# taohan10200/CRA5

Hardware: AMD Instinct MI355X
Metric: ERA5 frames/s (721x1440x268) encode+decode (higher is better)
Workload: dtype f32 (3xf16-split MFMA, fp32 accumulate)

## Files before the change

cra5_amd/csrc/attention_split_f16.hip:

```cpp
#include <hip/hip_runtime.h>
#include <math.h>
#include <stdlib.h>

#include "../../include/cra5_amd.h"
#include "split.h"

CRA5_RANGE_TU(attn)

typedef float f32x16 __attribute__((ext_vector_type(16)));
typedef _Float16 half8 __attribute__((ext_vector_type(8)));
typedef _Float16 half4 __attribute__((ext_vector_type(4)));
typedef __fp16 fp16x4 __attribute__((__vector_size__(4 * sizeof(__fp16))));
#if defined(__HIP_DEVICE_COMPILE__)
#define CRA5_TR_READ(P) \
  __builtin_bit_cast(half4, __builtin_amdgcn_ds_read_tr16_b64_v4f16((__attribute__((address_space(3))) fp16x4 *)(P)))
#else
#define CRA5_TR_READ(P) (*reinterpret_cast<const half4 *>(P))
#endif

namespace {

__device__ __forceinline__ int xcd_remap(int bid, int nb) {
  const int q = nb / 8, r = nb % 8;
  const int xcd = bid % 8, within = bid / 8;
  const int base = (xcd < r) ? xcd * (q + 1) : r * (q + 1) + (xcd - r) * q;
  return base + within;
}

struct WinGeom {
  int H, W, wh, ww, nwc;
};

__device__ __forceinline__ int token_of(const WinGeom &g, int wr, int wc, int t) {
  if (g.ww == g.W && g.wh == g.H) return t;
  const int r = t / g.ww, c = t - r * g.ww;
  const int gr = wr * g.wh + r, gc = wc * g.ww + c;
  return (gr < g.H && gc < g.W) ? gr * g.W + gc : -1;
}

#ifdef CRA5_ATTN_TRACE
__device__ unsigned long long g_attn_trace[6 * 8192];
#define CRA5_ATRACE(SLOT, VAL)                                                                          \
  if (threadIdx.x == 0 && atrace_idx < 8192) g_attn_trace[atrace_idx * 6 + (SLOT)] = (VAL);
#else
#define CRA5_ATRACE(SLOT, VAL)
#endif

constexpr int HD = 64;
constexpr int KS = 72;
constexpr int VS = 96;
constexpr int MAX_WIN_TOKENS = 1152;

struct BalArgs {
  int groups;
  int n_full;
  int n_wg_pass;
  int rem_tile0;
  int rem;
  int n_grp;
  int nkt;
  int maxp;
  float *ws;
};
__host__ __device__ __forceinline__ long bal_cut(long S, int G, int c) { return S * c / G; }
__host__ __device__ __forceinline__ int bal_piece_of(long S, int G, long s) {
  int c = (int)(s * G / S);
  if (c > G - 1) c = G - 1;
  while (c > 0 && bal_cut(S, G, c) > s) --c;
  while (c < G - 1 && bal_cut(S, G, c + 1) <= s) ++c;
  return c;
}
constexpr int WS_ROW = 68;

template <int NW, bool HI, bool GLOBAL, bool BAL = false, bool PLAIN = false>
__global__ __launch_bounds__(NW * 64, (NW >= 8 ? 1 : (NW == 4 ? 3 : 2))) void window_attention_split_kernel(
    const unsigned short *__restrict__ qkv, long ldq ,
    const unsigned short *__restrict__ pad_row, float *__restrict__ out, unsigned short *__restrict__ out_s,
    int Kp_out, int C, int heads, WinGeom g, int q_tiles , float scale, BalArgs bal) {
  static_assert(!BAL || GLOBAL, "the balanced schedule is for whole-grid launches");
  static_assert(!PLAIN || HI, "plain rows carry no lo plane");
  constexpr int NT = NW * 64;
  constexpr int PPR = PLAIN ? 8 : 16;
  constexpr int PIECES = 32 * PPR;
  constexpr int STG = (PIECES + NT - 1) / NT;

  constexpr int KPL = 32 * KS + 32;
  constexpr int VPL = 32 * VS;
  constexpr int KBUF = 2 * KPL, VBUF = 2 * VPL;
  __shared__ __attribute__((aligned(16))) unsigned short lds[2 * KBUF + 2 * VBUF];
  unsigned short *Ks = lds;
  unsigned short *Vt = lds + 2 * KBUF;
  constexpr int TAB = GLOBAL ? 1 : MAX_WIN_TOKENS;
  __shared__ long long tab[TAB];

  const int L = g.wh * g.ww;
  int head, win, n_seg = 1;
  int seg_tile0[2] = {0, 0}, seg_nact[2] = {NW, NW}, seg_j0[2] = {0, 0}, seg_j1[2] = {L / 32, L / 32}, seg_part[2] = {-1, -1};
  int seg_grp[2] = {0, 0};
  if (BAL) {
    const int pass = blockIdx.x / bal.n_wg_pass, w = blockIdx.x - pass * bal.n_wg_pass;
    int slot;
    if ((heads & 7) == 0 && (bal.n_wg_pass & 7) == 0) {
      const int xcd = w & 7, s_ = w >> 3;
      head = xcd * (heads >> 3) + s_ / bal.groups;
      slot = s_ % bal.groups;
    } else {
      head = w / bal.groups;
      slot = w % bal.groups;
    }
    win = 0;
    if (pass < bal.n_full) {
      seg_tile0[0] = (pass * bal.groups + slot) * NW;
    } else {
      const long S = (long)bal.n_grp * bal.nkt;
      const long s0 = bal_cut(S, bal.groups, slot), s1 = bal_cut(S, bal.groups, slot + 1);
      n_seg = 0;
      for (long s = s0; s < s1;) {
        const int gq = (int)(s / bal.nkt);
        const long e = min(s1, (long)(gq + 1) * bal.nkt);
        if (n_seg < 2) {
          seg_grp[n_seg] = gq;
          seg_tile0[n_seg] = bal.rem_tile0 + gq * NW;
          seg_nact[n_seg] = min(NW, bal.rem - gq * NW);
          seg_j0[n_seg] = (int)(s - (long)gq * bal.nkt);
          seg_j1[n_seg] = (int)(e - (long)gq * bal.nkt);
          seg_part[n_seg] = slot - bal_piece_of(S, bal.groups, (long)gq * bal.nkt);
          ++n_seg;
        }
        s = e;
      }
    }
  } else {
    const int pid = xcd_remap(blockIdx.x, gridDim.x);
    const int qt = pid % q_tiles;
    const int wh_id = pid / q_tiles;
    head = wh_id % heads;
    win = wh_id / heads;
    seg_tile0[0] = qt * NW;
  }
  const int wr = win / g.nwc, wc = win - wr * g.nwc;

  const int tid = threadIdx.x, lane = tid & 63, wave = tid >> 6;
  const int l31 = lane & 31, h = lane >> 5;
  const int hoff = head * HD;
  const long qoff = (PLAIN ? 1L : 2L) * hoff, koff = (PLAIN ? 1L : 2L) * (C + hoff), voff = (PLAIN ? 1L : 2L) * (2 * C + hoff);

  if (!GLOBAL) {
    const long long pad_delta = reinterpret_cast<const char *>(pad_row) - reinterpret_cast<const char *>(qkv);
    for (int t = tid; t < L; t += NT) {
      const int tok = token_of(g, wr, wc, t);
      tab[t] = (tok >= 0) ? (long long)tok * ldq * 2 : pad_delta;
    }
  }
  constexpr bool IDLE_SKIP = !GLOBAL || BAL;
  bool tab_ready = GLOBAL;
#pragma unroll 1
  for (int seg = 0; seg < n_seg; ++seg) {
  const int tile0 = seg_tile0[seg], n_active = seg_nact[seg], j0 = seg_j0[seg], j1 = seg_j1[seg];
#ifdef CRA5_ATTN_TRACE
  const int atrace_idx = GLOBAL ? 8192 : (int)blockIdx.x;
  const unsigned long long atrace_c0 = clock64();
#endif
  CRA5_ATRACE(0, wall_clock64());
  const int tq = (tile0 + wave) * 32 + l31;
  const int q_tok = (tq < L && wave < n_active) ? token_of(g, wr, wc, tq) : -1;
  const bool wave_active = __any(q_tok >= 0);
  if (!__syncthreads_or(wave_active ? 1 : 0)) continue;
  tab_ready = true;

  half8 qh[4], ql[4];
  {
    const unsigned short *qrow = ((q_tok >= 0) ? qkv + (size_t)q_tok * ldq : pad_row) + qoff;
#pragma unroll
    for (int s = 0; s < 4; ++s) {
      const int chunk = s >> 1, pp = 2 * (s & 1) + h;
      if (PLAIN) {
        qh[s] = *reinterpret_cast<const half8 *>(qrow + 16 * s + 8 * h);
        ql[s] = qh[s];
      } else {
        qh[s] = *reinterpret_cast<const half8 *>(qrow + chunk * 64 + pp * 8);
        ql[s] = *reinterpret_cast<const half8 *>(qrow + chunk * 64 + 32 + pp * 8);
      }
    }
  }
  const float cexp = scale * 1.44269504088896340736f;
  f32x16 negm;
#pragma unroll
  for (int r = 0; r < 16; ++r) negm[r] = 0.f;
  if (HI) {
#pragma unroll
    for (int s = 0; s < 4; ++s)
#pragma unroll
      for (int e = 0; e < 8; ++e) qh[s][e] = (_Float16)((float)qh[s][e] * cexp);
  }
  const float cmax = HI ? 1.0f : cexp;

  f32x16 o[2];
#pragma unroll
  for (int t = 0; t < 2; ++t)
#pragma unroll
    for (int r = 0; r < 16; ++r) o[t][r] = 0.f;
  float m_run = HI ? 0.f : -INFINITY, l_run = 0.f;

  const int n_tiles = j1 - j0;
  uint4 sk0 = make_uint4(0u, 0u, 0u, 0u), sk1 = sk0, sv0 = sk0, sv1 = sk0;
  static_assert(STG == 1 || STG == 2, "staging below is written out for one or two 16-byte pieces per thread");
  constexpr bool TWO = STG == 2;
  const int krow0 = min(tid / PPR, 31), krow1 = min((tid + NT) / PPR, 31);
  const long kcol = koff + (tid % PPR) * 8;
  const long vcol = voff + (tid % PPR) * 8;
  const unsigned short *kq0 = qkv + (size_t)(krow0 + 32 * j0) * ldq + kcol;
  const unsigned short *kq1 = qkv + (size_t)(krow1 + 32 * j0) * ldq + kcol;
  const unsigned short *vq0 = qkv + (size_t)(krow0 + 32 * j0) * ldq + vcol;
  const unsigned short *vq1 = qkv + (size_t)(krow1 + 32 * j0) * ldq + vcol;
  const long tile_step = 32 * ldq;
#define CRA5_ROW(JJ, ROW) \
  reinterpret_cast<const unsigned short *>(reinterpret_cast<const char *>(qkv) + tab[(JJ)*32 + (ROW)])
  const bool stage0 = (NT <= PIECES) || (tid < PIECES);
  const bool stage1 = TWO && (tid + NT < PIECES);
#define CRA5_K_LOAD(J)                                                                    \
  if (stage0) {                                                                           \
    if (GLOBAL) {                                                                         \
      sk0 = *reinterpret_cast<const uint4 *>(kq0);                                        \
      if (stage1) sk1 = *reinterpret_cast<const uint4 *>(kq1);                            \
      const long st_ = ((J) < n_tiles - 1) ? tile_step : 0;  \
      kq0 += st_;                                                                         \
      kq1 += st_;                                                                         \
    } else {                                                                              \
      const int jj_ = min((J), n_tiles - 1);                                              \
      sk0 = *reinterpret_cast<const uint4 *>(CRA5_ROW(jj_, krow0) + kcol);                \
      if (stage1) sk1 = *reinterpret_cast<const uint4 *>(CRA5_ROW(jj_, krow1) + kcol);    \
    }                                                                                     \
  }
#define CRA5_V_LOAD(J)                                                                    \
  if (stage0) {                                                                           \
    if (GLOBAL) {                                                                         \
      sv0 = *reinterpret_cast<const uint4 *>(vq0);                                        \
      if (stage1) sv1 = *reinterpret_cast<const uint4 *>(vq1);                            \
      const long st_ = ((J) < n_tiles - 1) ? tile_step : 0;                               \
      vq0 += st_;                                                                         \
      vq1 += st_;                                                                         \
    } else {                                                                              \
      const int jj_ = min((J), n_tiles - 1);                                              \
      sv0 = *reinterpret_cast<const uint4 *>(CRA5_ROW(jj_, krow0) + vcol);                \
      if (stage1) sv1 = *reinterpret_cast<const uint4 *>(CRA5_ROW(jj_, krow1) + vcol);    \
    }                                                                                     \
  }
#define CRA5_K_STORE1(P, BUF)                                                             \
  {                                                                                       \
    const int idx = tid + (P)*NT;                                                         \
    if (idx < PIECES) {                                                                   \
      const int row = idx / PPR, piece = idx % PPR;                                       \
      const int plane = PLAIN ? 0 : (piece >> 2) & 1, d0 = PLAIN ? 8 * piece : 32 * (piece >> 3) + 8 * (piece & 3); \
      *reinterpret_cast<uint4 *>(Ks + (BUF)*KBUF + plane * KPL + row * KS + d0) = sk##P;  \
    }                                                                                     \
  }
#define CRA5_K_STORE(BUF) { CRA5_K_STORE1(0, BUF) if (TWO) CRA5_K_STORE1(1, BUF) }
#define CRA5_V_STORE1(P, BUF)                                                             \
  {                                                                                       \
    const int idx = tid + (P)*NT;                                                         \
    if (idx < PIECES) {                                                                   \
      const int row = idx / PPR, piece = idx % PPR;                                       \
      const int plane = PLAIN ? 0 : (piece >> 2) & 1, d0 = PLAIN ? 8 * piece : 32 * (piece >> 3) + 8 * (piece & 3); \
      *reinterpret_cast<uint4 *>(Vt + (BUF)*VBUF + plane * VPL + row * VS + d0) = sv##P;  \
    }                                                                                     \
  }
#define CRA5_V_STORE(BUF) { CRA5_V_STORE1(0, BUF) if (TWO) CRA5_V_STORE1(1, BUF) }
#define CRA5_SCORES(DST, KB)                                                              \
  {                                                                                       \
    f32x16 acc_;                                                                          \
    _Pragma("unroll") for (int r = 0; r < 16; ++r) acc_[r] = 0.f;                         \
    _Pragma("unroll") for (int st = 0; st < 4; ++st) {                                    \
      const half8 kh = *reinterpret_cast<const half8 *>(k_base + (KB)*KBUF + 16 * st);     \
      const half8 kl = *reinterpret_cast<const half8 *>(k_base + (KB)*KBUF + KPL + 16 * st); \
      if (!HI) {                                                                          \
        acc_ = __builtin_amdgcn_mfma_f32_32x32x16_f16(kl, qh[st], acc_, 0, 0, 0);         \
        acc_ = __builtin_amdgcn_mfma_f32_32x32x16_f16(kh, ql[st], acc_, 0, 0, 0);         \
      }                                                                                   \
      if (HI && st == 0) {                                                                \
        CRA5_MFMA_FROM(acc_, kh, qh[0], negm);                                            \
      } else {                                                                            \
        acc_ = __builtin_amdgcn_mfma_f32_32x32x16_f16(kh, qh[st], acc_, 0, 0, 0);         \
      }                                                                                   \
    }                                                                                     \
    DST = acc_;                                                                           \
  }
#if defined(__HIP_DEVICE_COMPILE__)
#define CRA5_MFMA_FROM(D, A, B, C) \
  asm("s_nop 3\n\tv_mfma_f32_32x32x16_f16 %0, %1, %2, %3" : "=&v"(D) : "v"(A), "v"(B), "v"(C))
#else
#define CRA5_MFMA_FROM(D, A, B, C) (D) = (C)
#endif

  const unsigned short *k_base = Ks + l31 * KS + 8 * h;
  const unsigned short *v_base = Vt + (4 * h + ((lane & 15) >> 2)) * VS + 16 * ((lane >> 4) & 1) + 4 * (lane & 3);

#if defined(__HIP_DEVICE_COMPILE__)
#define CRA5_XHALF_MAX(X)                                                                 \
  ({                                                                                      \
    float a_ = (X), b_ = (X), r_;                                                         \
    asm("s_nop 1\n\tv_permlane32_swap_b32_e32 %0, %1\n\ts_nop 1\n\tv_max_f32_e32 %2, %0, %1" \
        : "+v"(a_), "+v"(b_), "=v"(r_));                                                  \
    r_;                                                                                   \
  })
#define CRA5_MAX2_VALU(A, B)                                                              \
  ({                                                                                      \
    float r_;                                                                             \
    asm("v_max_f32_e32 %0, %1, %2" : "=v"(r_) : "v"(A), "v"(B));                          \
    r_;                                                                                   \
  })
#else
#define CRA5_XHALF_MAX(X) (X)
#define CRA5_MAX2_VALU(A, B) fmaxf((A), (B))
#endif
#if !defined(__HIP_DEVICE_COMPILE__)
#define CRA5_TILE_MAX(S)                                                                  \
  ({                                                                                      \
    float m_ = fmaxf(fmaxf(fmaxf(S[0], S[1]), fmaxf(S[2], S[3])), fmaxf(fmaxf(S[4], S[5]), fmaxf(S[6], S[7]))); \
    float n_ = fmaxf(fmaxf(fmaxf(S[8], S[9]), fmaxf(S[10], S[11])), fmaxf(fmaxf(S[12], S[13]), fmaxf(S[14], S[15]))); \
    CRA5_XHALF_MAX(fmaxf(m_, n_)) * cmax;       \
  })
#else
#define CRA5_MAX3(A, B, C) fmaxf(fmaxf((A), (B)), (C))
#define CRA5_TILE_MAX(S)                                                                  \
  ({                                                                                      \
    const float a_ = CRA5_MAX3(S[0], S[1], S[2]), b_ = CRA5_MAX3(S[3], S[4], S[5]), c_ = CRA5_MAX3(S[6], S[7], S[8]); \
    const float d_ = CRA5_MAX3(S[9], S[10], S[11]), e_ = CRA5_MAX3(S[12], S[13], S[14]);     \
    const float f_ = CRA5_MAX3(a_, b_, c_), g_ = CRA5_MAX3(d_, e_, S[15]);                   \
    CRA5_XHALF_MAX(CRA5_MAX2_VALU(f_, g_)) * cmax;  \
  })
#endif

  f32x16 s_cur;
  CRA5_K_LOAD(0);
  CRA5_V_LOAD(0);
  CRA5_K_STORE(0);
  CRA5_V_STORE(0);
  CRA5_K_LOAD(1);
  CRA5_K_STORE(1);
  __syncthreads();
  CRA5_K_LOAD(2);
  CRA5_V_LOAD(1);
  CRA5_SCORES(s_cur, 0);
  float mloc = CRA5_TILE_MAX(s_cur);
  __syncthreads();

  auto key_tile = [&](const int j, f32x16 &s_cur, f32x16 &s_next) __attribute__((always_inline)) {
    const int kb = (j + 1) & 1, vb = j & 1;
    if (!IDLE_SKIP || wave_active) {
    constexpr float DEFER_LOG2 = 8.0f;
    auto shift = [&](float delta, const bool rescale, f32x16 *also) __attribute__((always_inline)) {
      delta = (float)(_Float16)fminf(fmaxf(delta, -60000.f), 60000.f);
      if (rescale) {
        const float alpha = __builtin_amdgcn_exp2f(-delta);
        l_run *= alpha;
#pragma unroll
        for (int t = 0; t < 2; ++t)
#pragma unroll
          for (int r = 0; r < 16; ++r) o[t][r] *= alpha;
      }
      m_run += delta;
      half8 e0, bd;
#pragma unroll
      for (int e = 0; e < 8; ++e) {
        e0[e] = (_Float16)0.0f;
        bd[e] = (_Float16)0.0f;
      }
      e0[0] = (_Float16)(h == 0 ? 1.0f : 0.0f);
      bd[0] = (_Float16)(h == 0 ? -delta : 0.0f);
      s_cur = __builtin_amdgcn_mfma_f32_32x32x16_f16(e0, bd, s_cur, 0, 0, 0);
      negm = __builtin_amdgcn_mfma_f32_32x32x16_f16(e0, bd, negm, 0, 0, 0);
      if (also) *also = __builtin_amdgcn_mfma_f32_32x32x16_f16(e0, bd, *also, 0, 0, 0);
#if defined(__HIP_DEVICE_COMPILE__)
      asm volatile("s_nop 15\n\ts_nop 3" ::: "memory");
#endif
    };
    if (HI) {
      if (j == 0) shift(mloc, false, nullptr);
    } else if (!__all(mloc - m_run <= DEFER_LOG2)) {
      const float m_new = fmaxf(m_run, mloc);
      const float alpha = __builtin_amdgcn_exp2f(m_run - m_new);
      l_run *= alpha;
#pragma unroll
      for (int t = 0; t < 2; ++t)
#pragma unroll
        for (int r = 0; r < 16; ++r) o[t][r] *= alpha;
      m_run = m_new;
    }
    const float m_new = m_run;
#if defined(__HIP_DEVICE_COMPILE__)
    if (!HI) {
#define CRA5_FENCE() __builtin_amdgcn_sched_barrier(0)
#define CRA5_STAGE(MFMA_STMT) \
  CRA5_FENCE();               \
  MFMA_STMT;                  \
  CRA5_FENCE();
#define CRA5_KFRAG(PLANE, ST) (*reinterpret_cast<const half8 *>(k_base + kb * KBUF + (PLANE)*KPL + 16 * (ST)))
#define CRA5_MM(A, B, C) __builtin_amdgcn_mfma_f32_32x32x16_f16((A), (B), (C), 0, 0, 0)
      typedef _Float16 half2v __attribute__((ext_vector_type(2)));
      typedef unsigned u32x4 __attribute__((ext_vector_type(4)));
      float p[16], psum = 0.f;
      u32x4 phw[2], plw[2];
      auto exp_half = [&](const int u) __attribute__((always_inline)) {
        p[2 * u] = __builtin_amdgcn_exp2f(fmaf(s_cur[2 * u], cexp, -m_new));
        p[2 * u + 1] = __builtin_amdgcn_exp2f(fmaf(s_cur[2 * u + 1], cexp, -m_new));
      };
      auto split_half = [&](const int u) __attribute__((always_inline)) {
        const int r = 2 * u;
        const half2v h2 = {(_Float16)p[r], (_Float16)p[r + 1]};
        const unsigned hh = __builtin_bit_cast(unsigned, h2);
        float d0, d1;
        asm("v_fma_mix_f32 %0, %2, -1.0, %3 op_sel_hi:[1,0,0]\n\t"
            "v_fma_mix_f32 %1, %2, -1.0, %4 op_sel:[1,0,0] op_sel_hi:[1,0,0]"
            : "=&v"(d0), "=&v"(d1) : "v"(hh), "v"(p[r]), "v"(p[r + 1]));
        psum += p[r];
        psum += p[r + 1];
        const half2v l2 = {(_Float16)d0, (_Float16)d1};
        unsigned ll = __builtin_bit_cast(unsigned, l2);
        asm("" : "+v"(ll));
        phw[u >> 2][u & 3] = hh;
        plw[u >> 2][u & 3] = ll;
      };
#define ph(T) __builtin_bit_cast(half8, phw[T])
#define pl(T) __builtin_bit_cast(half8, plw[T])
      half8 vh[2], vl[2];
      auto v_frag = [&](const int t, const int plane, const int dt) __attribute__((always_inline)) {
        const unsigned short *vp = v_base + vb * VBUF + plane * VPL + 16 * t * VS + 32 * dt;
        const half4 a0 = CRA5_TR_READ(vp);
        const half4 a1 = CRA5_TR_READ(vp + 8 * VS);
        return __builtin_shufflevector(a0, a1, 0, 1, 2, 3, 4, 5, 6, 7);
      };
      half8 kh0 = CRA5_KFRAG(0, 0), kl0 = CRA5_KFRAG(1, 0), kh1 = CRA5_KFRAG(0, 1), kl1 = CRA5_KFRAG(1, 1);
      f32x16 acc;
#pragma unroll
      for (int r = 0; r < 16; ++r) acc[r] = 0.f;
      CRA5_STAGE(acc = CRA5_MM(kl0, qh[0], acc))
      exp_half(0);
      CRA5_STAGE(acc = CRA5_MM(kh0, ql[0], acc))
      exp_half(1);
      CRA5_STAGE(acc = CRA5_MM(kh0, qh[0], acc))
      split_half(0);
      const half8 kh2 = CRA5_KFRAG(0, 2), kl2 = CRA5_KFRAG(1, 2);
      CRA5_STAGE(acc = CRA5_MM(kl1, qh[1], acc))
      exp_half(2);
      CRA5_STAGE(acc = CRA5_MM(kh1, ql[1], acc))
      split_half(1);
      CRA5_STAGE(acc = CRA5_MM(kh1, qh[1], acc))
      exp_half(3);
      const half8 kh3 = CRA5_KFRAG(0, 3), kl3 = CRA5_KFRAG(1, 3);
      CRA5_STAGE(acc = CRA5_MM(kl2, qh[2], acc))
      split_half(2);
      CRA5_STAGE(acc = CRA5_MM(kh2, ql[2], acc))
      exp_half(4);
      CRA5_STAGE(acc = CRA5_MM(kh2, qh[2], acc))
      split_half(3);
      CRA5_STAGE(acc = CRA5_MM(kl3, qh[3], acc))
      exp_half(5);
      vl[0] = v_frag(0, 1, 0);
      vl[1] = v_frag(0, 1, 1);
      CRA5_STAGE(acc = CRA5_MM(kh3, ql[3], acc))
      split_half(4);
      CRA5_STAGE(acc = CRA5_MM(kh3, qh[3], acc))
      split_half(5);
      vh[0] = v_frag(0, 0, 0);
      vh[1] = v_frag(0, 0, 1);
      s_next = acc;
      CRA5_STAGE(o[0] = CRA5_MM(vl[0], ph(0), o[0]))
      exp_half(6);
      CRA5_STAGE(o[1] = CRA5_MM(vl[1], ph(0), o[1]))
      exp_half(7);
      CRA5_STAGE(o[0] = CRA5_MM(vh[0], pl(0), o[0]))
      split_half(6);
      CRA5_STAGE(o[1] = CRA5_MM(vh[1], pl(0), o[1]))
      split_half(7);
      vl[0] = v_frag(1, 1, 0);
      vl[1] = v_frag(1, 1, 1);
      CRA5_STAGE(o[0] = CRA5_MM(vh[0], ph(0), o[0]))
      l_run += psum;
      CRA5_STAGE(o[1] = CRA5_MM(vh[1], ph(0), o[1]))
      vh[0] = v_frag(1, 0, 0);
      vh[1] = v_frag(1, 0, 1);
      CRA5_STAGE(o[0] = CRA5_MM(vl[0], ph(1), o[0]))
      const float ma = CRA5_MAX3(s_next[0], s_next[1], s_next[2]), mb = CRA5_MAX3(s_next[3], s_next[4], s_next[5]);
      const float mc = CRA5_MAX3(s_next[6], s_next[7], s_next[8]), md = CRA5_MAX3(s_next[9], s_next[10], s_next[11]);
      const float me = CRA5_MAX3(s_next[12], s_next[13], s_next[14]);
      CRA5_STAGE(o[1] = CRA5_MM(vl[1], ph(1), o[1]))
      const float mf = CRA5_MAX3(ma, mb, mc), mg = CRA5_MAX3(md, me, s_next[15]);
      const float mfg = CRA5_MAX2_VALU(mf, mg);
      CRA5_STAGE(o[0] = CRA5_MM(vh[0], pl(1), o[0]))
      const float mx = CRA5_XHALF_MAX(mfg);
      CRA5_STAGE(o[1] = CRA5_MM(vh[1], pl(1), o[1]))
      mloc = mx * cmax;
      CRA5_STAGE(o[0] = CRA5_MM(vh[0], ph(1), o[0]))
      CRA5_STAGE(o[1] = CRA5_MM(vh[1], ph(1), o[1]))
#undef ph
#undef pl
#undef CRA5_MM
#undef CRA5_KFRAG
#undef CRA5_STAGE
#undef CRA5_FENCE
    } else
#endif
    {
    CRA5_SCORES(s_next, kb);
    float psum = 0.f;
    half8 ph[2], pl[2];
#if defined(__HIP_DEVICE_COMPILE__)
    if (HI) {
      typedef _Float16 half2v __attribute__((ext_vector_type(2)));
      typedef _Float16 half8v __attribute__((ext_vector_type(8)));
      const half2v ones = {(_Float16)1.0f, (_Float16)1.0f};
      auto exps = [&]() __attribute__((always_inline)) {
        psum = 0.f;
#pragma unroll
        for (int t = 0; t < 2; ++t) {
          half2v hp[4];
#pragma unroll
          for (int i = 0; i < 4; ++i) {
            hp[i] = half2v{(_Float16)__builtin_amdgcn_exp2f(s_cur[8 * t + 2 * i]), (_Float16)__builtin_amdgcn_exp2f(s_cur[8 * t + 2 * i + 1])};
            psum = __builtin_amdgcn_fdot2(hp[i], ones, psum, false);
          }
          ph[t] = half8v{hp[0][0], hp[0][1], hp[1][0], hp[1][1], hp[2][0], hp[2][1], hp[3][0], hp[3][1]};
        }
      };
      exps();
      constexpr float P_SAFE = 8192.0f;
      if (!__all(psum <= P_SAFE)) {
        const float mrel = CRA5_TILE_MAX(s_cur);
        shift(fmaxf(mrel, 0.f), true, &s_next);
        exps();
      }
#pragma unroll
      for (int t = 0; t < 2; ++t)
#pragma unroll
        for (int e = 0; e < 8; ++e) pl[t][e] = (_Float16)0.0f;
    }
#else
#pragma unroll
    for (int r = 0; r < 16; ++r) {
      const float p = HI ? (float)(_Float16)__builtin_amdgcn_exp2f(s_cur[r]) : __builtin_amdgcn_exp2f(fmaf(s_cur[r], cexp, -m_new));
      psum += p;
      const _Float16 hi = (_Float16)p;
      const _Float16 lo = (_Float16)(p - (float)hi);
      ph[r >> 3][r & 7] = hi;
      pl[r >> 3][r & 7] = lo;
    }
#endif
    l_run += psum;
#pragma unroll
    for (int t = 0; t < 2; ++t) {
      half8 vh[2], vl[2];
#pragma unroll
      for (int dt = 0; dt < 2; ++dt) {
        const unsigned short *vp = v_base + vb * VBUF + 16 * t * VS + 32 * dt;
        const unsigned short *vq = vp + VPL;
        const half4 a0 = CRA5_TR_READ(vp);
        const half4 a1 = CRA5_TR_READ(vp + 8 * VS);
        const half4 b0 = CRA5_TR_READ(vq);
        const half4 b1 = CRA5_TR_READ(vq + 8 * VS);
        vh[dt] = __builtin_shufflevector(a0, a1, 0, 1, 2, 3, 4, 5, 6, 7);
        vl[dt] = __builtin_shufflevector(b0, b1, 0, 1, 2, 3, 4, 5, 6, 7);
      }
      if (!HI) {
        o[0] = __builtin_amdgcn_mfma_f32_32x32x16_f16(vl[0], ph[t], o[0], 0, 0, 0);
        o[1] = __builtin_amdgcn_mfma_f32_32x32x16_f16(vl[1], ph[t], o[1], 0, 0, 0);
        o[0] = __builtin_amdgcn_mfma_f32_32x32x16_f16(vh[0], pl[t], o[0], 0, 0, 0);
        o[1] = __builtin_amdgcn_mfma_f32_32x32x16_f16(vh[1], pl[t], o[1], 0, 0, 0);
      }
      o[0] = __builtin_amdgcn_mfma_f32_32x32x16_f16(vh[0], ph[t], o[0], 0, 0, 0);
      o[1] = __builtin_amdgcn_mfma_f32_32x32x16_f16(vh[1], ph[t], o[1], 0, 0, 0);
    }
    if (!HI) mloc = CRA5_TILE_MAX(s_next);
    }
    }
    CRA5_K_STORE(j & 1);
    CRA5_V_STORE((j + 1) & 1);
    CRA5_K_LOAD(j + 3);
    CRA5_V_LOAD(j + 2);
    __syncthreads();
  };
  CRA5_ATRACE(1, wall_clock64());
  f32x16 s_alt;
  const int n_loop = n_tiles;
  int jt = 0;
  for (; jt + 1 < n_loop; jt += 2) {
    key_tile(jt, s_cur, s_alt);
    key_tile(jt + 1, s_alt, s_cur);
  }
  if (jt < n_loop) key_tile(jt, s_cur, s_alt);
  CRA5_ATRACE(2, wall_clock64());
  CRA5_ATRACE(4, (unsigned long long)n_tiles);

  const float l_tot = l_run + __shfl_xor(l_run, 32, 64);
  if (BAL && seg_part[seg] >= 0) {
    if (q_tok >= 0) {
      float *wrow = bal.ws + (((((size_t)head * bal.n_grp + seg_grp[seg]) * bal.maxp + seg_part[seg]) * NW + wave) * 32 + l31) * WS_ROW;
#pragma unroll
      for (int t = 0; t < 2; ++t)
#pragma unroll
        for (int gq = 0; gq < 4; ++gq) {
          const int d = 32 * t + 8 * gq + 4 * h;
          *reinterpret_cast<float4 *>(wrow + d) = make_float4(o[t][4 * gq + 0], o[t][4 * gq + 1], o[t][4 * gq + 2], o[t][4 * gq + 3]);
        }
      if (h == 0) {
        wrow[64] = m_run;
        wrow[65] = l_tot;
      }
    }
    continue;
  }
  {
    const bool live = q_tok >= 0;
    const float inv = live ? 1.0f / l_tot : 0.0f;
    float *orow = (out && live) ? out + (size_t)q_tok * C + hoff : nullptr;
    unsigned short *srow = (out_s && live) ? out_s + (size_t)q_tok * 2 * Kp_out : nullptr;
#pragma unroll
    for (int t = 0; t < 2; ++t)
#pragma unroll
      for (int pr = 0; pr < 2; ++pr) {
        float va[4], vb[4];
#pragma unroll
        for (int k = 0; k < 4; ++k) {
          va[k] = o[t][4 * (2 * pr) + k] * inv;
          vb[k] = o[t][4 * (2 * pr + 1) + k] * inv;
        }
        if (orow) {
          *reinterpret_cast<float4 *>(orow + 32 * t + 16 * pr + 4 * h) = make_float4(va[0], va[1], va[2], va[3]);
          *reinterpret_cast<float4 *>(orow + 32 * t + 16 * pr + 8 + 4 * h) = make_float4(vb[0], vb[1], vb[2], vb[3]);
        }
        if (out_s) {
          unsigned ha0, la0, ha1, la1, hb0, lb0, hb1, lb1;
          cra5_split_pair(va[0], va[1], ha0, la0);
          cra5_split_pair(va[2], va[3], ha1, la1);
          cra5_split_pair(vb[0], vb[1], hb0, lb0);
          cra5_split_pair(vb[2], vb[3], hb1, lb1);
#if defined(__HIP_DEVICE_COMPILE__)
#define CRA5_SWAP32(A, B)                                                  \
  {                                                                        \
    const auto r_ = __builtin_amdgcn_permlane32_swap((A), (B), false, false); \
    (A) = r_[0];                                                           \
    (B) = r_[1];                                                           \
  }
          CRA5_SWAP32(ha0, hb0);
          CRA5_SWAP32(ha1, hb1);
          CRA5_SWAP32(la0, lb0);
          CRA5_SWAP32(la1, lb1);
#undef CRA5_SWAP32
#endif
          if (srow) {
            const int c0 = hoff + 32 * t + 16 * pr + 8 * h;
            unsigned short *sp = srow + (PLAIN ? c0 : (c0 >> 5) * 64 + (c0 & 31));
            *reinterpret_cast<uint4 *>(sp) = make_uint4(ha0, ha1, hb0, hb1);
            if (!HI) *reinterpret_cast<uint4 *>(sp + 32) = make_uint4(la0, la1, lb0, lb1);
          }
        }
      }
  }
  CRA5_ATRACE(3, wall_clock64());
  CRA5_ATRACE(5, clock64() - atrace_c0);
  }
  (void)tab_ready;
}

__global__ __launch_bounds__(256) void attention_merge_kernel(const float *__restrict__ ws, float *__restrict__ out,
                                                              unsigned short *__restrict__ out_s, int Kp_out, int C,
                                                              BalArgs bal, int nw, int plain) {
  const int t = blockIdx.x % nw, hg = blockIdx.x / nw;
  const int grp = hg % bal.n_grp, head = hg / bal.n_grp;
  if (grp * nw + t >= bal.rem) return;
  const long S = (long)bal.n_grp * bal.nkt;
  const int c0 = bal_piece_of(S, bal.groups, (long)grp * bal.nkt);
  const int c1 = bal_piece_of(S, bal.groups, (long)(grp + 1) * bal.nkt - 1);
  const int np = c1 - c0 + 1;
  const int q = threadIdx.x >> 3, d0 = (threadIdx.x & 7) * 8;
  const size_t pstride = (size_t)nw * 32 * WS_ROW;
  const float *base = ws + ((((size_t)head * bal.n_grp + grp) * bal.maxp) * nw + t) * 32 * WS_ROW + (size_t)q * WS_ROW;
  float M = -INFINITY;
  for (int c = 0; c < np; ++c) M = fmaxf(M, base[c * pstride + 64]);
  float acc[8] = {0.f, 0.f, 0.f, 0.f, 0.f, 0.f, 0.f, 0.f}, lsum = 0.f;
  for (int c = 0; c < np; ++c) {
    const float *r = base + c * pstride;
    const float a = __builtin_amdgcn_exp2f(r[64] - M);
    lsum = fmaf(r[65], a, lsum);
    const float4 v0 = *reinterpret_cast<const float4 *>(r + d0), v1 = *reinterpret_cast<const float4 *>(r + d0 + 4);
    acc[0] = fmaf(v0.x, a, acc[0]);
    acc[1] = fmaf(v0.y, a, acc[1]);
    acc[2] = fmaf(v0.z, a, acc[2]);
    acc[3] = fmaf(v0.w, a, acc[3]);
    acc[4] = fmaf(v1.x, a, acc[4]);
    acc[5] = fmaf(v1.y, a, acc[5]);
    acc[6] = fmaf(v1.z, a, acc[6]);
    acc[7] = fmaf(v1.w, a, acc[7]);
  }
  const float inv = 1.0f / lsum;
  const int tok = (bal.rem_tile0 + grp * nw + t) * 32 + q, col = head * HD + d0;
#pragma unroll
  for (int k = 0; k < 8; ++k) acc[k] *= inv;
  if (out) {
    *reinterpret_cast<float4 *>(out + (size_t)tok * C + col) = make_float4(acc[0], acc[1], acc[2], acc[3]);
    *reinterpret_cast<float4 *>(out + (size_t)tok * C + col + 4) = make_float4(acc[4], acc[5], acc[6], acc[7]);
  }
  if (out_s) {
    unsigned short *srow = out_s + (size_t)tok * 2 * Kp_out;
    if (plain) {
      cra5_store_plain4(srow, col, acc[0], acc[1], acc[2], acc[3]);
      cra5_store_plain4(srow, col + 4, acc[4], acc[5], acc[6], acc[7]);
    } else {
      cra5_store_split4(srow, col, acc[0], acc[1], acc[2], acc[3]);
      cra5_store_split4(srow, col + 4, acc[4], acc[5], acc[6], acc[7]);
    }
  }
}

int cu_count() {
  static const int n = [] {
    int dev = 0, v = 0;
    if (hipGetDevice(&dev) != hipSuccess) return 256;
    if (hipDeviceGetAttribute(&v, hipDeviceAttributeMultiprocessorCount, dev) != hipSuccess || v <= 0) return 256;
    return v;
  }();
  return n;
}

constexpr int NW_GLOBAL = 12;

bool balanced_plan(int L, int heads, BalArgs &b) {
  const int P = cu_count(), T = L / 32;
  if (P % heads) return false;
  b.groups = P / heads;
  b.n_full = T / (b.groups * NW_GLOBAL);
  b.rem_tile0 = b.n_full * b.groups * NW_GLOBAL;
  b.rem = T - b.rem_tile0;
  b.n_grp = (b.rem + NW_GLOBAL - 1) / NW_GLOBAL;
  b.nkt = T;
  b.n_wg_pass = heads * b.groups;
  b.ws = nullptr;
  b.maxp = 0;
  const long S = (long)b.n_grp * b.nkt;
  for (int g = 0; g < b.n_grp; ++g) {
    const int np = bal_piece_of(S, b.groups, (long)(g + 1) * b.nkt - 1) - bal_piece_of(S, b.groups, (long)g * b.nkt) + 1;
    if (np > b.maxp) b.maxp = np;
  }
  if (!(b.n_full >= 1 && (b.rem == 0 || (b.n_grp <= b.groups && S >= b.groups)))) return false;
  for (int c = 0; b.rem && c < b.groups; ++c) {
    const long s0 = bal_cut(S, b.groups, c), s1 = bal_cut(S, b.groups, c + 1);
    if (s1 > s0 && (s1 - 1) / b.nkt - s0 / b.nkt + 1 > 2) return false;
  }
  return true;
}

size_t balanced_ws_bytes(const BalArgs &b, int heads) {
  return (size_t)heads * b.n_grp * b.maxp * NW_GLOBAL * 32 * WS_ROW * sizeof(float);
}

template <bool HI, bool PLAIN = false>
int launch_balanced(const unsigned short *qkv, long ldq, const unsigned short *pad_row, float *out, unsigned short *out_s,
                    int Kp_out, int C, int heads, int H, int W, float scale, BalArgs b, float *ws, hipStream_t st) {
  WinGeom g;
  g.H = H;
  g.W = W;
  g.wh = H;
  g.ww = W;
  g.nwc = 1;
  b.ws = ws;
  const int n_pass = b.n_full + (b.rem ? 1 : 0);
  hipLaunchKernelGGL((window_attention_split_kernel<NW_GLOBAL, HI, true, true, PLAIN>), dim3(n_pass * b.n_wg_pass),
                     dim3(NW_GLOBAL * 64), 0, st, qkv, ldq, pad_row, out, out_s, Kp_out, C, heads, g, 0, scale, b);
  int rc = (int)hipGetLastError();
  if (rc || b.rem == 0) return rc;
  hipLaunchKernelGGL(attention_merge_kernel, dim3(heads * b.n_grp * NW_GLOBAL), dim3(256), 0, st, ws, out, out_s, Kp_out,
                     C, b, NW_GLOBAL, PLAIN ? 1 : 0);
  return (int)hipGetLastError();
}

template <int NW, bool HI, bool GLOBAL, bool PLAIN = false>
int launch(const unsigned short *qkv, long ldq, const unsigned short *pad_row, float *out, unsigned short *out_s,
           int Kp_out, int C, int heads, int H, int W, int wh, int ww, float scale, hipStream_t st) {
  WinGeom g;
  g.H = H;
  g.W = W;
  g.wh = wh;
  g.ww = ww;
  const int nwr = (H + wh - 1) / wh;
  g.nwc = (W + ww - 1) / ww;
  const int L = wh * ww;
  const int q_tiles = (L + NW * 32 - 1) / (NW * 32);
  hipLaunchKernelGGL((window_attention_split_kernel<NW, HI, GLOBAL, false, PLAIN>), dim3(q_tiles * nwr * g.nwc * heads), dim3(NW * 64), 0, st,
                     qkv, ldq, pad_row, out, out_s, Kp_out, C, heads, g, q_tiles, scale, BalArgs{});
  return (int)hipGetLastError();
}

}

static int attention_dispatch(const uint16_t *qkv_split, int qkv_kp, const uint16_t *pad_row_split, float *out,
                              uint16_t *out_split, int out_kp, int C, int heads, int H, int W, int wh, int ww,
                              float scale, int mode, void *workspace, size_t workspace_bytes, void *stream,
                              bool want_balanced) {
  if (!qkv_split || !pad_row_split || (!out && !out_split) || heads <= 0 || C % heads) return CRA5_ERR_ARG;
  if (C / heads != 64 || qkv_kp != 3 * C) return CRA5_ERR_ARG;
  if (wh <= 0 || ww <= 0 || H <= 0 || W <= 0 || (wh * ww) % 32) return CRA5_ERR_ARG;
  if (out_split && (out_kp < C || out_kp % 32)) return CRA5_ERR_ARG;
  if (((uintptr_t)qkv_split & 15) || ((uintptr_t)pad_row_split & 15)) return CRA5_ERR_ARG;
  hipStream_t st = (hipStream_t)stream;
  const int L = wh * ww;
  constexpr int PLAIN_ROWS = CRA5_GEMM_HI_ONLY | CRA5_GEMM_A_PLAIN | CRA5_GEMM_OUT_PLAIN;
  if (mode != 0 && mode != CRA5_GEMM_HI_ONLY && mode != PLAIN_ROWS) return CRA5_ERR_ARG;
  const bool hi_only = mode != 0, plain = mode == PLAIN_ROWS;
  const long ldq = 2L * qkv_kp;
  const bool whole = (wh == H && ww == W);
  if (!whole && L > MAX_WIN_TOKENS) return CRA5_ERR_ARG;
#define CRA5_ATT_GO(NWV, HIV, GLV) \
  return launch<NWV, HIV, GLV>(qkv_split, ldq, pad_row_split, out, out_split, out_kp, C, heads, H, W, wh, ww, scale, st)
  if (whole) {
    BalArgs b;
    if (want_balanced && balanced_plan(L, heads, b) &&
        (balanced_ws_bytes(b, heads) == 0 ||
         (workspace && ((uintptr_t)workspace & 15) == 0 && workspace_bytes >= balanced_ws_bytes(b, heads)))) {
      float *ws = reinterpret_cast<float *>(workspace);
      if (plain)
        return launch_balanced<true, true>(qkv_split, ldq, pad_row_split, out, out_split, out_kp, C, heads, H, W, scale, b, ws, st);
      if (hi_only)
        return launch_balanced<true>(qkv_split, ldq, pad_row_split, out, out_split, out_kp, C, heads, H, W, scale, b, ws, st);
      return launch_balanced<false>(qkv_split, ldq, pad_row_split, out, out_split, out_kp, C, heads, H, W, scale, b, ws, st);
    }
    if (plain) return launch<NW_GLOBAL, true, true, true>(qkv_split, ldq, pad_row_split, out, out_split, out_kp, C, heads, H, W, wh, ww, scale, st);
    if (hi_only) CRA5_ATT_GO(NW_GLOBAL, true, true);
    CRA5_ATT_GO(NW_GLOBAL, false, true);
  }
  if (plain) return launch<4, true, false, true>(qkv_split, ldq, pad_row_split, out, out_split, out_kp, C, heads, H, W, wh, ww, scale, st);
  if (hi_only) CRA5_ATT_GO(4, true, false);
  CRA5_ATT_GO(4, false, false);
#undef CRA5_ATT_GO
}

#ifdef CRA5_ATTN_TRACE
extern "C" int cra5_debug_attn_trace(unsigned long long *host, int n_rows) {
  if (n_rows < 1 || n_rows > 8192) return CRA5_ERR_ARG;
  if (hipDeviceSynchronize() != hipSuccess) return CRA5_ERR_ARG;
  int rc = (int)hipMemcpyFromSymbol(host, HIP_SYMBOL(g_attn_trace), sizeof(unsigned long long) * 6 * n_rows);
  void *p = nullptr;
  if (hipGetSymbolAddress(&p, HIP_SYMBOL(g_attn_trace)) == hipSuccess) hipMemset(p, 0, sizeof(unsigned long long) * 6 * 8192);
  return rc;
}
#endif

extern "C" int cra5_window_attention_split(const uint16_t *qkv_split, int qkv_kp, const uint16_t *pad_row_split,
                                           float *out, uint16_t *out_split, int out_kp, int C, int heads, int H,
                                           int W, int wh, int ww, float scale, int mode, void *stream) {
  return attention_dispatch(qkv_split, qkv_kp, pad_row_split, out, out_split, out_kp, C, heads, H, W, wh, ww, scale,
                            mode, nullptr, 0, stream, false);
}

extern "C" size_t cra5_attention_workspace_bytes(int n_tokens, int heads) {
  BalArgs b;
  if (n_tokens <= 0 || heads <= 0 || (n_tokens % 32) || !balanced_plan(n_tokens, heads, b)) return 0;
  return balanced_ws_bytes(b, heads);
}

extern "C" int cra5_window_attention_split_ws(const uint16_t *qkv_split, int qkv_kp, const uint16_t *pad_row_split,
                                              float *out, uint16_t *out_split, int out_kp, int C, int heads, int H,
                                              int W, int wh, int ww, float scale, int mode, void *workspace,
                                              size_t workspace_bytes, void *stream) {
  return attention_dispatch(qkv_split, qkv_kp, pad_row_split, out, out_split, out_kp, C, heads, H, W, wh, ww, scale,
                            mode, workspace, workspace_bytes, stream, true);
}

extern "C" int cra5_attention_balanced_plan(int n_tokens, int heads, size_t *workspace_bytes) {
  BalArgs b;
  if (workspace_bytes) *workspace_bytes = 0;
  if (n_tokens <= 0 || heads <= 0 || (n_tokens % 32) || !balanced_plan(n_tokens, heads, b)) return 0;
  if (workspace_bytes) *workspace_bytes = balanced_ws_bytes(b, heads);
  return 1;
}
```

Baseline: 32.33.

## Interleave K/V staging and barrier inside windowed attention key-tile pipeline

For the non-HI, non-global (windowed) attention variant, the K/V global loads, LDS stores and the block barrier move from the end of each key tile into the middle of the MFMA schedule, using a targeted vmcnt wait and a raw s_barrier in place of __syncthreads. The final tile gets a specialised LAST path that skips computing next-tile scores and the max, and idle waves run a lightweight staging-only loop. Bounds checks on staging are removed when the piece count divides evenly. The goal is to hide load and barrier latency behind matrix math, at the cost of more complex scheduling and a risk of ordering hazards from the hand-placed waitcnt.

```diff
diff --git a/cra5_amd/csrc/attention_split_f16.hip b/cra5_amd/csrc/attention_split_f16.hip
--- a/cra5_amd/csrc/attention_split_f16.hip
+++ b/cra5_amd/csrc/attention_split_f16.hip
@@ -45,6 +45,11 @@
 #else
 #define CRA5_ATRACE(SLOT, VAL)
 #endif
+
+template <bool B>
+struct BoolC {
+  static constexpr bool value = B;
+};
 
 constexpr int HD = 64;
 constexpr int KS = 72;
@@ -153,6 +158,11 @@
     }
   }
   constexpr bool IDLE_SKIP = !GLOBAL || BAL;
+#if defined(__HIP_DEVICE_COMPILE__)
+  constexpr bool MID = !HI && !GLOBAL;
+#else
+  constexpr bool MID = false;
+#endif
   bool tab_ready = GLOBAL;
 #pragma unroll 1
   for (int seg = 0; seg < n_seg; ++seg) {
@@ -217,7 +227,7 @@
 #define CRA5_ROW(JJ, ROW) \
   reinterpret_cast<const unsigned short *>(reinterpret_cast<const char *>(qkv) + tab[(JJ)*32 + (ROW)])
   const bool stage0 = (NT <= PIECES) || (tid < PIECES);
-  const bool stage1 = TWO && (tid + NT < PIECES);
+  const bool stage1 = TWO && ((MID && 2 * NT <= PIECES) || tid + NT < PIECES);
 #define CRA5_K_LOAD(J)                                                                    \
   if (stage0) {                                                                           \
     if (GLOBAL) {                                                                         \
@@ -249,7 +259,7 @@
 #define CRA5_K_STORE1(P, BUF)                                                             \
   {                                                                                       \
     const int idx = tid + (P)*NT;                                                         \
-    if (idx < PIECES) {                                                                   \
+    if ((MID && (P + 1) * NT <= PIECES) || idx < PIECES) {  \
       const int row = idx / PPR, piece = idx % PPR;                                       \
       const int plane = PLAIN ? 0 : (piece >> 2) & 1, d0 = PLAIN ? 8 * piece : 32 * (piece >> 3) + 8 * (piece & 3); \
       *reinterpret_cast<uint4 *>(Ks + (BUF)*KBUF + plane * KPL + row * KS + d0) = sk##P;  \
@@ -259,7 +269,7 @@
 #define CRA5_V_STORE1(P, BUF)                                                             \
   {                                                                                       \
     const int idx = tid + (P)*NT;                                                         \
-    if (idx < PIECES) {                                                                   \
+    if ((MID && (P + 1) * NT <= PIECES) || idx < PIECES) {  \
       const int row = idx / PPR, piece = idx % PPR;                                       \
       const int plane = PLAIN ? 0 : (piece >> 2) & 1, d0 = PLAIN ? 8 * piece : 32 * (piece >> 3) + 8 * (piece & 3); \
       *reinterpret_cast<uint4 *>(Vt + (BUF)*VBUF + plane * VPL + row * VS + d0) = sv##P;  \
@@ -331,23 +341,40 @@
   })
 #endif
 
+#if defined(__HIP_DEVICE_COMPILE__)
+#define CRA5_STAGED_ARRIVED() __builtin_amdgcn_s_waitcnt(0x0F70)
+#define CRA5_TILE_BARRIER()                               \
+  {                                                       \
+    __builtin_amdgcn_sched_barrier(0);                    \
+    asm volatile("s_waitcnt lgkmcnt(0)" ::: "memory");    \
+    __builtin_amdgcn_s_barrier();                         \
+    asm volatile("" ::: "memory");                        \
+    __builtin_amdgcn_sched_barrier(0);                    \
+  }
+#else
+#define CRA5_TILE_BARRIER() __syncthreads()
+#define CRA5_STAGED_ARRIVED()
+#endif
   f32x16 s_cur;
   CRA5_K_LOAD(0);
   CRA5_V_LOAD(0);
   CRA5_K_STORE(0);
   CRA5_V_STORE(0);
-  CRA5_K_LOAD(1);
-  CRA5_K_STORE(1);
+  if (!MID || n_tiles > 1) {
+    CRA5_K_LOAD(1);
+    CRA5_K_STORE(1);
+  }
   __syncthreads();
-  CRA5_K_LOAD(2);
-  CRA5_V_LOAD(1);
+  if (!MID || n_tiles > 2) { CRA5_K_LOAD(2); }
+  if (!MID || n_tiles > 1) { CRA5_V_LOAD(1); }
   CRA5_SCORES(s_cur, 0);
   float mloc = CRA5_TILE_MAX(s_cur);
   __syncthreads();
 
-  auto key_tile = [&](const int j, f32x16 &s_cur, f32x16 &s_next) __attribute__((always_inline)) {
+  auto key_tile = [&](const int j, f32x16 &s_cur, f32x16 &s_next, auto last_c) __attribute__((always_inline)) {
+    constexpr bool LAST = decltype(last_c)::value;
     const int kb = (j + 1) & 1, vb = j & 1;
-    if (!IDLE_SKIP || wave_active) {
+    if (MID || !IDLE_SKIP || wave_active) {
     constexpr float DEFER_LOG2 = 8.0f;
     auto shift = [&](float delta, const bool rescale, f32x16 *also) __attribute__((always_inline)) {
       delta = (float)(_Float16)fminf(fmaxf(delta, -60000.f), 60000.f);
@@ -430,6 +457,7 @@
         const half4 a1 = CRA5_TR_READ(vp + 8 * VS);
         return __builtin_shufflevector(a0, a1, 0, 1, 2, 3, 4, 5, 6, 7);
       };
+      if (!LAST) {
       half8 kh0 = CRA5_KFRAG(0, 0), kl0 = CRA5_KFRAG(1, 0), kh1 = CRA5_KFRAG(0, 1), kl1 = CRA5_KFRAG(1, 1);
       f32x16 acc;
 #pragma unroll
@@ -448,23 +476,60 @@
       CRA5_STAGE(acc = CRA5_MM(kh1, qh[1], acc))
       exp_half(3);
       const half8 kh3 = CRA5_KFRAG(0, 3), kl3 = CRA5_KFRAG(1, 3);
+      if (MID) {
+        CRA5_STAGED_ARRIVED();
+        if (j + 2 < n_tiles) { CRA5_K_STORE(j & 1); }
+      }
       CRA5_STAGE(acc = CRA5_MM(kl2, qh[2], acc))
       split_half(2);
       CRA5_STAGE(acc = CRA5_MM(kh2, ql[2], acc))
       exp_half(4);
       CRA5_STAGE(acc = CRA5_MM(kh2, qh[2], acc))
       split_half(3);
+      if (MID) { CRA5_TILE_BARRIER(); }
       CRA5_STAGE(acc = CRA5_MM(kl3, qh[3], acc))
       exp_half(5);
       vl[0] = v_frag(0, 1, 0);
       vl[1] = v_frag(0, 1, 1);
+      if (MID) { CRA5_V_STORE((j + 1) & 1); }
       CRA5_STAGE(acc = CRA5_MM(kh3, ql[3], acc))
       split_half(4);
+      if (MID && j + 3 < n_tiles) { CRA5_K_LOAD(j + 3); }
       CRA5_STAGE(acc = CRA5_MM(kh3, qh[3], acc))
       split_half(5);
       vh[0] = v_frag(0, 0, 0);
       vh[1] = v_frag(0, 0, 1);
+      if (MID && j + 2 < n_tiles) { CRA5_V_LOAD(j + 2); }
       s_next = acc;
+      } else {
+      exp_half(0);
+      CRA5_FENCE();
+      exp_half(1);
+      CRA5_FENCE();
+      split_half(0);
+      CRA5_FENCE();
+      exp_half(2);
+      CRA5_FENCE();
+      split_half(1);
+      CRA5_FENCE();
+      exp_half(3);
+      CRA5_FENCE();
+      split_half(2);
+      CRA5_FENCE();
+      exp_half(4);
+      CRA5_FENCE();
+      split_half(3);
+      CRA5_TILE_BARRIER();
+      exp_half(5);
+      vl[0] = v_frag(0, 1, 0);
+      vl[1] = v_frag(0, 1, 1);
+      CRA5_FENCE();
+      split_half(4);
+      CRA5_FENCE();
+      split_half(5);
+      vh[0] = v_frag(0, 0, 0);
+      vh[1] = v_frag(0, 0, 1);
+      }
       CRA5_STAGE(o[0] = CRA5_MM(vl[0], ph(0), o[0]))
       exp_half(6);
       CRA5_STAGE(o[1] = CRA5_MM(vl[1], ph(0), o[1]))
@@ -480,6 +545,7 @@
       CRA5_STAGE(o[1] = CRA5_MM(vh[1], ph(0), o[1]))
       vh[0] = v_frag(1, 0, 0);
       vh[1] = v_frag(1, 0, 1);
+      if (!LAST) {
       CRA5_STAGE(o[0] = CRA5_MM(vl[0], ph(1), o[0]))
       const float ma = CRA5_MAX3(s_next[0], s_next[1], s_next[2]), mb = CRA5_MAX3(s_next[3], s_next[4], s_next[5]);
       const float mc = CRA5_MAX3(s_next[6], s_next[7], s_next[8]), md = CRA5_MAX3(s_next[9], s_next[10], s_next[11]);
@@ -491,6 +557,12 @@
       const float mx = CRA5_XHALF_MAX(mfg);
       CRA5_STAGE(o[1] = CRA5_MM(vh[1], pl(1), o[1]))
       mloc = mx * cmax;
+      } else {
+      CRA5_STAGE(o[0] = CRA5_MM(vl[0], ph(1), o[0]))
+      CRA5_STAGE(o[1] = CRA5_MM(vl[1], ph(1), o[1]))
+      CRA5_STAGE(o[0] = CRA5_MM(vh[0], pl(1), o[0]))
+      CRA5_STAGE(o[1] = CRA5_MM(vh[1], pl(1), o[1]))
+      }
       CRA5_STAGE(o[0] = CRA5_MM(vh[0], ph(1), o[0]))
       CRA5_STAGE(o[1] = CRA5_MM(vh[1], ph(1), o[1]))
 #undef ph
@@ -573,21 +645,47 @@
     if (!HI) mloc = CRA5_TILE_MAX(s_next);
     }
     }
-    CRA5_K_STORE(j & 1);
-    CRA5_V_STORE((j + 1) & 1);
-    CRA5_K_LOAD(j + 3);
-    CRA5_V_LOAD(j + 2);
-    __syncthreads();
+    if (!MID) {
+      CRA5_K_STORE(j & 1);
+      CRA5_V_STORE((j + 1) & 1);
+      CRA5_K_LOAD(j + 3);
+      CRA5_V_LOAD(j + 2);
+      __syncthreads();
+    }
   };
   CRA5_ATRACE(1, wall_clock64());
   f32x16 s_alt;
-  const int n_loop = n_tiles;
   int jt = 0;
-  for (; jt + 1 < n_loop; jt += 2) {
-    key_tile(jt, s_cur, s_alt);
-    key_tile(jt + 1, s_alt, s_cur);
-  }
-  if (jt < n_loop) key_tile(jt, s_cur, s_alt);
+  if (MID && IDLE_SKIP && !wave_active) {
+#pragma unroll 1
+    for (int j = 0; j < n_tiles; ++j) {
+      CRA5_STAGED_ARRIVED();
+      if (j + 2 < n_tiles) { CRA5_K_STORE(j & 1); }
+      CRA5_TILE_BARRIER();
+      if (j + 1 < n_tiles) { CRA5_V_STORE((j + 1) & 1); }
+      if (j + 3 < n_tiles) { CRA5_K_LOAD(j + 3); }
+      if (j + 2 < n_tiles) { CRA5_V_LOAD(j + 2); }
+    }
+  } else if (MID) {
+    for (; jt + 2 < n_tiles; jt += 2) {
+      key_tile(jt, s_cur, s_alt, BoolC<false>{});
+      key_tile(jt + 1, s_alt, s_cur, BoolC<false>{});
+    }
+    if (jt + 1 < n_tiles) {
+      key_tile(jt, s_cur, s_alt, BoolC<false>{});
+      s_cur = s_alt;
+      ++jt;
+    }
+    key_tile(jt, s_cur, s_alt, BoolC<true>{});
+  } else {
+    for (; jt + 1 < n_tiles; jt += 2) {
+      key_tile(jt, s_cur, s_alt, BoolC<false>{});
+      key_tile(jt + 1, s_alt, s_cur, BoolC<false>{});
+    }
+    if (jt < n_tiles) key_tile(jt, s_cur, s_alt, BoolC<false>{});
+  }
+#undef CRA5_TILE_BARRIER
+#undef CRA5_STAGED_ARRIVED
   CRA5_ATRACE(2, wall_clock64());
   CRA5_ATRACE(4, (unsigned long long)n_tiles);
 
```

New measurement: 32.40, median of 2. Within noise of the previous version (+0.2%).
